# j-moralejo-pinas/dist_classicrl

Hardware: AMD Instinct MI355X
Metric: env-steps/sec at 128 agents, 1e6x16 Q-table; 1/2/4/8 GPU + HBM GB/s %peak (higher is better)
Workload: dtype f32

## Files before the change

### dist_classicrl_amd/csrc/qe_inst_lane.hip

```cpp
#include "qe_host.h"
#include "qe_rollout_df.h"

#if !defined(QE_INST_T) || !defined(QE_INST_ENV)
#error "compile with -DQE_INST_T=<float|double> -DQE_INST_ENV=<HashEnv|GridEnv|BanditEnv|TttEnv|TableEnv>"
#endif

template <int NV, int CAP, bool MK, int LEAN, bool HELP, bool FULL, bool SEQ>
constexpr int64_t lane_variant() {
    return QE_VARIANT_PERSISTENT | ((int64_t)LEAN << 4) | ((int64_t)HELP << 6) | ((int64_t)FULL << 7) | ((int64_t)SEQ << 8) |
           ((int64_t)(CAP == LANE_MAX_AGENTS) << 9) | ((int64_t)NV << 12) | ((int64_t)MK << 20);
}

template <typename T, class Env>
int launch_persistent(qe_engine* e, qe_env* env, RolloutSlot& sl, const Ctx<T>& c, const EnvCtx& ev, int64_t steps, int mode,
                      int build) {
    const unsigned block = (unsigned)((env->N + 63) / 64 * 64);
    int flags = FLAG_ACCOUNT;
#ifdef QE_EXPERIMENT
    if (getenv("QE_DEBUG_FLAGS")) flags |= atoi(getenv("QE_DEBUG_FLAGS")) << 20;
#endif
    const bool lean = mode == QE_LEARN_ITER && !c.trace && !c.rp.s;
    auto go = [&](auto nv, auto masked) {
        constexpr int NV = decltype(nv)::value;
        constexpr bool MK = decltype(masked)::value;
        constexpr bool HAS_LEAN = std::is_same<T, float>::value &&
                                  ((std::is_same<Env, HashEnv>::value && !MK && (NV == 2 || NV == 4)) ||
                                   std::is_same<Env, TttEnv>::value);
        const bool full = (int64_t)block == env->N;
        const bool light = build == 1, sparse = build == 3;
        auto launch = [&](auto cap, auto lean_c, auto help, auto full_c, auto seq, unsigned threads) {
            constexpr int CAP = decltype(cap)::value, LEAN = decltype(lean_c)::value;
            constexpr bool HELP = decltype(help)::value, FULL = decltype(full_c)::value, SEQ = decltype(seq)::value;
            hipLaunchKernelGGL((k_rollout_lane<T, Env, NV, CAP, MK, LEAN, HELP, FULL, SEQ>), dim3(1), dim3(threads), 0, e->stream,
                               sl.sched, c, ev, (long long)steps, flags);
            sl.variant = lane_variant<NV, CAP, MK, LEAN, HELP, FULL, SEQ>();
        };
        auto launch_df = [&](auto lean_c, auto full_c) {
            constexpr int LEAN = decltype(lean_c)::value;
            constexpr bool FULL = decltype(full_c)::value;
            if constexpr (LEAN != 0) {
                hipLaunchKernelGGL((k_rollout_df<T, Env, NV, MK, LEAN, FULL>), dim3(1), dim3(2 * block), 0, e->stream,
                                   sl.sched, c, ev, (long long)steps, flags);
                sl.variant = lane_variant<NV, 128, MK, LEAN, true, FULL, true>() | QE_VARIANT_DATAFLOW;
            }
        };
        using I128 = std::integral_constant<int, 128>;
        using I512 = std::integral_constant<int, LANE_MAX_AGENTS>;
        using L0 = std::integral_constant<int, 0>;
        using L1 = std::integral_constant<int, HAS_LEAN ? 1 : 0>;
        using L2 = std::integral_constant<int, HAS_LEAN ? 2 : 0>;
        using Y = std::integral_constant<bool, HAS_LEAN>;
        using N = std::false_type;
        auto by_lean = [&](auto f) { if (c.dlog) f(L2{}); else f(L1{}); };
        if (HAS_LEAN && lean && block <= 128) {
            if (full && sparse) by_lean([&](auto l) { launch(I128{}, l, Y{}, Y{}, Y{}, 2 * block); });
            else if (full && light) by_lean([&](auto l) { launch_df(l, Y{}); });
            else if (light) by_lean([&](auto l) { launch_df(l, N{}); });
            else if (full) by_lean([&](auto l) { launch(I128{}, l, Y{}, Y{}, N{}, std::max(512u, 2 * block)); });
            else by_lean([&](auto l) { launch(I128{}, l, Y{}, N{}, N{}, std::max(512u, 2 * block)); });
        } else {
            launch(I512{}, L0{}, N{}, N{}, N{}, block);
        }
    };
    using Yes = std::true_type;
    using No = std::false_type;
    if constexpr (std::is_same<Env, HashEnv>::value || std::is_same<Env, TableEnv>::value) {
        auto by_mask = [&](auto nv) { if (env->p.masked) go(nv, Yes{}); else go(nv, No{}); };
        switch (e->ld) {
            case 4: by_mask(std::integral_constant<int, 1>{}); break;
            case 8: by_mask(std::integral_constant<int, 2>{}); break;
            case 16: by_mask(std::integral_constant<int, 4>{}); break;
            case 32: by_mask(std::integral_constant<int, 8>{}); break;
            default: by_mask(std::integral_constant<int, 16>{}); break;
        }
    } else if constexpr (std::is_same<Env, TttEnv>::value) {
        go(std::integral_constant<int, 4>{}, Yes{});
    } else {
        go(std::integral_constant<int, 1>{}, No{});
    }
    ++sl.launches;
    return QE_OK;
}

template int launch_persistent<QE_INST_T, QE_INST_ENV>(qe_engine*, qe_env*, RolloutSlot&, const Ctx<QE_INST_T>&, const EnvCtx&, int64_t, int,
                                                       int);
```

### dist_classicrl_amd/csrc/qe_rollout_lane.h

```cpp
#pragma once
#include "qe_kernels.h"

namespace qe {

constexpr int LANE_MAX_AGENTS = 512;

template <typename T, int NV>
struct RowV {
    T v[4 * NV];
};

template <int NV>
struct LaneMask {
    using type = uint32_t;
};
template <>
struct LaneMask<16> {
    using type = uint64_t;
};

__device__ __forceinline__ int popc_mask(uint32_t x) { return __popc(x); }
__device__ __forceinline__ int popc_mask(uint64_t x) { return __popcll(x); }

template <int NV>
__device__ __forceinline__ void load_row_lane(RowV<float, NV>& r, const float* q, int64_t row) {
    const float4* p = reinterpret_cast<const float4*>(q + row * (4 * NV));
#pragma unroll
    for (int k = 0; k < NV; ++k) {
        const float4 f = p[k];
        r.v[4 * k] = f.x; r.v[4 * k + 1] = f.y; r.v[4 * k + 2] = f.z; r.v[4 * k + 3] = f.w;
    }
}
template <int NV>
__device__ __forceinline__ void load_row_lane(RowV<double, NV>& r, const double* q, int64_t row) {
    const double2* p = reinterpret_cast<const double2*>(q + row * (4 * NV));
#pragma unroll
    for (int k = 0; k < NV; ++k) {
        const double2 a = p[2 * k], b = p[2 * k + 1];
        r.v[4 * k] = a.x; r.v[4 * k + 1] = a.y; r.v[4 * k + 2] = b.x; r.v[4 * k + 3] = b.y;
    }
}

__device__ __forceinline__ float lane_fmax(float a, float b) { return __builtin_fmaxf(a, b); }
__device__ __forceinline__ double lane_fmax(double a, double b) { return __builtin_fmax(a, b); }

template <bool MASKED, typename T, int NV, typename M>
__device__ __forceinline__ RowV<T, NV> masked_row(const RowV<T, NV>& row, M valid) {
    if constexpr (!MASKED) {
        return row;
    } else {
        RowV<T, NV> r;
#pragma unroll
        for (int j = 0; j < 4 * NV; ++j) r.v[j] = ((valid >> j) & 1) ? row.v[j] : neg_inf<T>();
        return r;
    }
}

template <typename T, int NV>
__device__ __forceinline__ T row_max_lane(const RowV<T, NV>& rowm) {
    T m = neg_inf<T>();
#pragma unroll
    for (int j = 0; j < 4 * NV; ++j) m = lane_fmax(m, rowm.v[j]);
    return m;
}

template <int NV>
__device__ __forceinline__ bool row_nan_lane(const RowV<float, NV>& rowm) {
    typedef float f2 __attribute__((ext_vector_type(2)));
    f2 acc0 = {0.0f, 0.0f}, acc1 = {0.0f, 0.0f};
#pragma unroll
    for (int j = 0; j < 4 * NV; j += 4) {
        const f2 x = {rowm.v[j], rowm.v[j + 1]}, y = {rowm.v[j + 2], rowm.v[j + 3]};
        acc0 = __builtin_elementwise_fma(x, x, acc0);
        acc1 = __builtin_elementwise_fma(y, y, acc1);
    }
    const f2 acc = acc0 + acc1;
    const float s = acc.x + acc.y;
    return s != s;
}
template <int NV>
__device__ __forceinline__ bool row_nan_lane(const RowV<double, NV>& rowm) {
    double acc = 0.0;
#pragma unroll
    for (int j = 0; j < 4 * NV; ++j) acc += rowm.v[j] * rowm.v[j];
    return acc != acc;
}
template <typename T, int NV>
__device__ __forceinline__ T row_max_np_lane(const RowV<T, NV>& rowm) {
    const T m = row_max_lane(rowm);
    return row_nan_lane<NV>(rowm) ? quiet_nan<T>() : m;
}

template <typename T, int NV, int LO, int CNT>
__device__ __forceinline__ T row_pick_tree(const RowV<T, NV>& row, int idx) {
    constexpr int W = 4 * NV;
    if constexpr (CNT == 1) {
        T x = row.v[LO < W ? LO : W - 1];
        asm volatile("" : "+v"(x));
        return x;
    } else {
        const T lo = row_pick_tree<T, NV, LO, CNT / 2>(row, idx);
        const T hi = row_pick_tree<T, NV, LO + CNT / 2, CNT / 2>(row, idx);
        T r = (idx & (CNT / 2)) ? hi : lo;
        asm volatile("" : "+v"(r));
        return r;
    }
}
template <typename T, int NV>
__device__ __forceinline__ T row_pick_lane(const RowV<T, NV>& row, int idx) {
    constexpr int W = 4 * NV;
    constexpr int P = W <= 4 ? 4 : (W <= 8 ? 8 : (W <= 16 ? 16 : (W <= 32 ? 32 : 64)));
    return row_pick_tree<T, NV, 0, P>(row, idx);
}

template <int NV, typename M>
__device__ __forceinline__ int kth_set_bit(M f, int k) {
    constexpr int W = 4 * NV;
    constexpr int P = W <= 4 ? 4 : (W <= 8 ? 8 : (W <= 16 ? 16 : (W <= 32 ? 32 : 64)));
    constexpr int LOG = P == 4 ? 2 : (P == 8 ? 3 : (P == 16 ? 4 : (P == 32 ? 5 : 6)));
    int pos = 0;
#pragma unroll
    for (int lv = 0; lv < LOG; ++lv) {
        const int width = P >> (lv + 1);
        const M low = f & (((M)1 << width) - 1);
        const int c = popc_mask(low);
        const bool hi = k >= c;
        k -= hi ? c : 0;
        f = hi ? (f >> width) : low;
        pos += hi ? width : 0;
    }
    return pos;
}

template <typename T, int NV, typename M>
__device__ __forceinline__ int select_lane(const RowV<T, NV>& rowm, M valid, bool explore, uint32_t x1,
                                           uint32_t x2, T* picked, bool nan_max) {
    T m = row_max_lane(rowm);
    if (nan_max) m = quiet_nan<T>();
    M ties = 0;
#pragma unroll
    for (int j = 0; j < 4 * NV; ++j) ties |= (M)(rowm.v[j] == m ? 1u : 0u) << j;
    const M f = explore ? valid : (ties & valid);
    const int total = popc_mask(f);
    int act = -1;
    if (total > 0) act = kth_set_bit<NV>(f, (int)mulhi32(explore ? x1 : x2, (uint32_t)total));
    *picked = row_pick_lane(rowm, act < 0 ? 0 : act);
    return act;
}

template <class Env, int NV, bool MASKED>
__device__ __forceinline__ typename LaneMask<NV>::type valid_mask_lane(const EnvCtx& ev, int64_t i, int32_t obs) {
    using M = typename LaneMask<NV>::type;
    if constexpr (!MASKED) {
        return ev.A >= 8 * (int)sizeof(M) ? ~(M)0 : (((M)1 << ev.A) - 1);
    } else {
        M m = 0;
#pragma unroll
        for (int sub = 0; sub < NV; ++sub) m |= (M)Env::valid4(ev, i, obs, sub) << (4 * sub);
        return m;
    }
}

template <int CAP>
struct LaneCfg {
    static constexpr int WT = CAP <= 128 ? 4096 : 2048;
    static constexpr int BT = 2048;
};

template <int CAP, bool HELP>
struct LaneLds {
    SlowLdsT<CAP, PERSIST_CACHE_BYTES> slow;
    int wt[4][LaneCfg<CAP>::WT + 1];
    int bt_key[LaneCfg<CAP>::BT];
    unsigned bt_cnt[LaneCfg<CAP>::BT];
    int bt_min[LaneCfg<CAP>::BT];
    uint32_t draws[2][3][HELP ? CAP : 1];
    unsigned long long ep_key[EP_STAGE];
    float ep_ret[EP_STAGE];
    unsigned char pending[CAP];
    alignas(16) unsigned char cold[448];
    unsigned def_bits[CAP / 32];
    unsigned busy[5];
    unsigned ep_n;
    unsigned n_def;
    unsigned complex_;
    int seq_min[2];
};

#ifdef QE_EXPERIMENT
#define QX(bit) ((flags >> (20 + (bit))) & 1)
#else
#define QX(bit) 0
#endif
#ifdef QE_STAMPS
#define QL_STAMP(k) do { const long long _n = wall_clock64(); stamp_sum[k] += _n - stamp_last; stamp_last = _n; } while (0)
#else
#define QL_STAMP(k) do { } while (0)
#endif

template <int PENDING_LOADS>
__device__ __forceinline__ void step_barrier() {
    if constexpr (PENDING_LOADS == 0) asm volatile("s_waitcnt vmcnt(0) lgkmcnt(0)\n\ts_barrier" ::: "memory");
    else asm volatile("s_waitcnt vmcnt(%0) lgkmcnt(0)\n\ts_barrier" ::"n"(PENDING_LOADS) : "memory");
}

template <typename T, class Env, int NV, int CAP, bool MASKED, int LEAN = 0, bool HELP = false, bool FULL = false,
          bool SEQ = false>
__global__ __launch_bounds__(HELP ? 4 * CAP : CAP) void k_rollout_lane(InlineSched ,
                                                                       Ctx<T> c, EnvCtx ev, long long steps, int flags) {
    using M = typename LaneMask<NV>::type;
    constexpr int NLOAD = NV * (int)(sizeof(T) / 4);
    constexpr int WT = LaneCfg<CAP>::WT, BT = LaneCfg<CAP>::BT;
    __shared__ LaneLds<CAP, HELP> lds;
    const unsigned long long clk0 = wall_clock64();
    const unsigned long long cyc0 = __builtin_amdgcn_s_memtime();
    if (c.thr == nullptr) {
        const QE_AS4 unsigned char* ka = (const QE_AS4 unsigned char*)__builtin_amdgcn_kernarg_segment_ptr();
        c.thr = (const QE_AS4 unsigned long long*)ka;
        c.lr = (const QE_AS4 double*)(ka + sizeof(unsigned long long) * INLINE_SCHED_STEPS);
    }
    if constexpr (LEAN != 0) { c.mode = 0; c.trace = nullptr; c.rp.s = nullptr; }
    if constexpr (LEAN == 1) c.dlog = nullptr;
#ifdef QE_STAMPS
    long long stamp_sum[8] = {0, 0, 0, 0, 0, 0, 0, 0};
    long long stamp_last = wall_clock64();
    if (threadIdx.x == 0) for (int k = 8; k < 24; ++k) c.vinc[k] = 0.0;
#endif
    const int tid = threadIdx.x;
    const int n_main = HELP ? (int)((c.N + 63) & ~63ll) : (int)blockDim.x;
    const int wave_tid = __builtin_amdgcn_readfirstlane(tid);
    const bool helper = HELP && wave_tid >= n_main && wave_tid < 2 * n_main;
    const bool worker = HELP && wave_tid >= 2 * n_main;
    const int i = helper ? tid - n_main : (worker ? 0 : tid);
    const bool active = FULL ? !(helper || worker) : (!(helper || worker) && i < c.N);
    const int ii = i < c.N ? i : 0;
    Pending<T> p;
    p.n = c.n[ii];
    p.aux = c.aux[ii];
    p.s = 0; p.a = 0; p.pred = 0; p.r = 0.0f; p.term = false;
    float acc = c.acc[ii];
    unsigned long long deferred_total = 0, ep_base = 0;
    unsigned complex_steps = 0;
    int w_next = WT, w_cur = WT, w_prev = WT;
    const int flush_every = 32;
    int flush_in = flush_every;
    for (int k = tid; k < 4 * (WT + 1); k += (int)blockDim.x) (&lds.wt[0][0])[k] = -1;
    for (int k = tid; k < BT; k += (int)blockDim.x) { lds.bt_key[k] = -1; lds.bt_cnt[k] = 0u; lds.bt_min[k] = 0x7FFFFFFF; }
    for (int k = tid; k < CAP; k += (int)blockDim.x) lds.pending[k] = 0;
    if (tid < CAP / 32) lds.def_bits[tid] = 0u;
    static_assert(sizeof(Ctx<T>) <= sizeof(lds.cold), "context stash too small");
    if (tid == 0) {
        *reinterpret_cast<Ctx<T>*>(lds.cold) = c;
        lds.ep_n = 0u; lds.n_def = 0u; lds.complex_ = 0u;
        lds.seq_min[0] = 0x7FFFFFFF; lds.seq_min[1] = 0x7FFFFFFF;
        for (int k = 0; k < 5; ++k) lds.busy[k] = 0u;
        c.ctrl->error = 0u;
        c.ctrl->inv_count = 0u;
    }
    __syncthreads();
    if ((QX(6) && worker) || (QX(7) && helper)) return;

    const bool nan_sel = c.nan_select != 0;
    auto advance = [&](const RowV<T, NV>& row, M valid, long long t1, const U4& x, unsigned long long thr_t1, bool row_nan) {
        const bool explore = (unsigned long long)x.x < thr_t1;
        T picked;
        int act = select_lane<T, NV, M>(masked_row<MASKED>(row, valid), valid, explore, x.y, x.z, &picked, nan_sel && row_nan);
        if (act < 0) {
            c.ctrl->error = ERR_EMPTY_CHOICE;
            act = 0;
        }
        const int32_t n = p.n;
        const Transition tr = Env::step(ev, i, n, p.aux, act, c.step0 + (unsigned long long)t1);
        if (c.trace) c.trace[t1 * c.N + i] = act;
        replay_put(c, t1, i, n, act, tr.reward, tr.next_obs, tr.terminated);
        p.s = n; p.a = act; p.pred = picked; p.r = tr.reward; p.term = tr.terminated; p.n = tr.next_obs;
    };
    auto philox_of = [&](long long t1) {
        const unsigned long long step1 = c.step0 + (unsigned long long)t1;
        return philox4x32_10(c.agent_offset + (uint32_t)ii, (uint32_t)step1, (uint32_t)(step1 >> 32), STREAM_POLICY,
                             c.seed_lo, c.seed_hi);
    };
    auto draws = [&](long long t1) {
        if constexpr (HELP) {
            const int slot = (int)(t1 & 1);
            return U4{lds.draws[slot][0][ii], lds.draws[slot][1][ii], lds.draws[slot][2][ii], 0u};
        } else {
            return philox_of(t1);
        }
    };
    auto produce = [&](long long t1) {
        const U4 x = philox_of(t1);
        const int slot = (int)(t1 & 1);
        lds.draws[slot][0][ii] = x.x; lds.draws[slot][1][ii] = x.y; lds.draws[slot][2][ii] = x.z;
    };
    auto bookkeeping = [&](long long k, bool check_stale) {
        int* const tab_w = lds.wt[(k + 1) & 3];
        const int* const tab_r = lds.wt[k & 3];
        const int* const tab_st = lds.wt[(k + 3) & 3];
        const int32_t rowid = p.n;
        const int h = (int)(mix32((uint32_t)rowid) & (WT - 1));
        const bool need_r = rowid != p.s;
        int o_w = atomicCAS(&tab_w[h], -1, rowid);
        int k_r = need_r ? tab_r[h] : -1;
        int k_st = check_stale ? tab_st[h] : -1;
        int h_w = h, h_r = h, h_st = h;
        bool odd_w = o_w != -1 && o_w != rowid, odd_r = k_r != -1 && k_r != rowid, odd_st = k_st != -1 && k_st != rowid;
        while (__any(odd_w || odd_r || odd_st)) {
            h_w = odd_w ? (h_w + 1) & (WT - 1) : h_w;
            h_r = (h_r + 1) & (WT - 1);
            h_st = (h_st + 1) & (WT - 1);
            const int o2 = atomicCAS(&tab_w[odd_w ? h_w : WT], odd_w ? -1 : -2, rowid);
            const int r2 = tab_r[odd_r ? h_r : WT];
            const int s2 = tab_st[odd_st ? h_st : WT];
            o_w = odd_w ? o2 : o_w; k_r = odd_r ? r2 : k_r; k_st = odd_st ? s2 : k_st;
            odd_w = o_w != -1 && o_w != rowid; odd_r = k_r != -1 && k_r != rowid; odd_st = k_st != -1 && k_st != rowid;
        }
        lds.busy[o_w == rowid ? (int)((k + 1) & 3) : 4] = 1u;
        lds.busy[k_r == rowid ? (int)(k & 3) : 4] = 1u;
        w_prev = w_cur; w_cur = w_next; w_next = h_w;
        return k_st == rowid;
    };

    RowV<T, NV> row;
    bool stale = false;
    {
        load_row_lane<NV>(row, c.q, p.n);
        if (active) {
            const M valid0 = valid_mask_lane<Env, NV, MASKED>(ev, i, p.n);
            advance(row, valid0, 0, philox_of(0), c.thr[0], row_nan_lane<NV>(masked_row<MASKED>(row, valid0)));
            int h = (int)(mix32((uint32_t)p.s) & (WT - 1));
            int old = atomicCAS(&lds.wt[0][h], -1, p.s);
            while (old != -1 && old != p.s) {
                h = (h + 1) & (WT - 1);
                old = atomicCAS(&lds.wt[0][h], -1, p.s);
            }
            if (old == p.s) lds.busy[0] = 1u;
            w_next = h;
        }
        if (helper) produce(1);
        __syncthreads();
        if (active) (void)bookkeeping(0, false);
        load_row_lane<NV>(row, c.q, p.n);
    }
    __syncthreads();
    DeltaEntry* dl = c.dlog ? c.dlog + c.dlog_base + ii : nullptr;
    const long long dl_steps = c.dlog ? (c.dlog_cap - c.dlog_base) / c.N : 0;
    int vzero;
    asm volatile("v_mov_b32 %0, 0" : "=v"(vzero));
    double lr_pend = ((const double*)(uintptr_t)c.lr)[vzero];
    unsigned long long thr_pend = ((const unsigned long long*)(uintptr_t)c.thr)[(steps > 1 ? 1 : 0) + vzero];
    for (long long t = 0; t < steps; ++t) {
        const bool last = t + 1 == steps;
        const bool dl_ok = t < dl_steps;
        QL_STAMP(7);
        const bool busy = lds.busy[t & 3] != 0u;
        const U4 x = draws(t + 1);
        if (helper && !last && !QX(5)) produce(t + 2);
        if (stale && !QX(8)) load_row_lane<NV>(row, c.q, p.n);
        const M valid = valid_mask_lane<Env, NV, MASKED>(ev, ii, p.n);
        QL_STAMP(0);
        int cls = 3;
        int pred_s = -1, pred_n = -1;
        int b_s = -1, b_n = -1;
        if (busy) {
            if (active) {
                auto bt_insert = [&](int32_t rowid) {
                    int h = (int)(mix32((uint32_t)rowid) & (BT - 1));
                    for (;;) {
                        const int old = atomicCAS(&lds.bt_key[h], -1, rowid);
                        if (old == -1 || old == rowid) return h;
                        h = (h + 1) & (BT - 1);
                    }
                };
                b_s = bt_insert(p.s);
                atomicAdd(&lds.bt_cnt[b_s], 1u << 16);
                atomicMin(&lds.bt_min[b_s], i);
                if (p.n != p.s) {
                    b_n = bt_insert(p.n);
                    atomicAdd(&lds.bt_cnt[b_n], 1u);
                    atomicMin(&lds.bt_min[b_n], i);
                }
            }
            barrier_lds();
            if (active) {
                const unsigned cs = lds.bt_cnt[b_s];
                const int ms = lds.bt_min[b_s];
                unsigned cn = 0u;
                int mn = 0x7FFFFFFF;
                const bool has_n = b_n >= 0;
                if (has_n) { cn = lds.bt_cnt[b_n]; mn = lds.bt_min[b_n]; }
                const unsigned w_s = cs >> 16, tot_s = w_s + (cs & 0xFFFFu);
                const unsigned w_n = cn >> 16, tot_n = w_n + (cn & 0xFFFFu);
                bool now = true, sel = true, cx = false;
                if (c.mode == 1) {
                    const bool shared = w_s >= 2u || (w_s == 1u && tot_s >= 2u) || (has_n && w_n >= 1u && tot_n >= 2u);
                    if (shared) { now = false; cx = true; }
                    sel = !(has_n ? w_n > 0u : w_s > 1u);
                } else {
                    if (tot_s > 1u && ms < i) { now = false; pred_s = ms; cx |= tot_s > 2u; }
                    if (has_n) {
                        if (w_n > 0u) {
                            sel = false;
                            if (!p.term && mn < i) { now = false; pred_n = mn; cx |= tot_n > 2u; }
                        }
                    } else if (w_s > 1u) {
                        sel = false;
                    }
                }
                cls = (now ? 1 : 0) | (sel ? 2 : 0);
                if (!now) {
                    lds.pending[i] = 1;
                    atomicAdd(&lds.n_def, 1u);
                    if (cx) lds.complex_ = 1u;
                }
            }
        }
        QL_STAMP(2);
        __builtin_amdgcn_s_waitcnt(0x0F70);
        double lr_t;
        unsigned long long thr_t1;
        asm volatile("v_mov_b64 %0, %1" : "=v"(lr_t) : "v"(lr_pend));
        asm volatile("v_mov_b64 %0, %1" : "=v"(thr_t1) : "v"(thr_pend));
        lr_pend = ((const double*)(uintptr_t)c.lr)[(last ? t : t + 1) + vzero];
        thr_pend = ((const unsigned long long*)(uintptr_t)c.thr)[(t + 2 < steps ? t + 2 : steps - 1) + vzero];
        const float r_t = p.r;
        const bool term_t = p.term;
        bool row_nan = row_nan_lane<NV>(masked_row<MASKED>(row, valid));
        if (active && (cls & 1)) {
            T m = row_max_lane(masked_row<MASKED>(row, valid));
            if (row_nan) m = quiet_nan<T>();
            const int64_t cell = (int64_t)p.s * (4 * NV) + p.a;
            T u;
            const T q1 = Td<T>::apply(p.pred, p.r, m, p.term, make_hyper(c, lr_t), c.mode, &u);
            if (p.n == p.s) row_nan |= q1 != q1;
            if (!QX(1)) c.q[cell] = q1;
            if (dl_ok) *dl = DeltaEntry{(uint32_t)cell, (float)u};
            if (p.n == p.s) {
#pragma unroll
                for (int j = 0; j < 4 * NV; ++j) row.v[j] = j == p.a ? q1 : row.v[j];
            }
        }
        unsigned ep_raw = 0;
        unsigned long long enders = 0;
        float ep_value = 0.0f;
        if (active) {
            acc += r_t;
            enders = __ballot(term_t && (flags & FLAG_ACCOUNT));
            const unsigned rank = __builtin_amdgcn_mbcnt_hi((unsigned)(enders >> 32), __builtin_amdgcn_mbcnt_lo((unsigned)enders, 0u));
            if (term_t) {
                if (rank == 0) ep_raw = atomicAdd(&lds.ep_n, (unsigned)__popcll(enders));
                ep_value = acc;
                acc = 0.0f;
            }
        }
        QL_STAMP(4);
        if (active && !busy && !last) advance(row, valid, t + 1, x, thr_t1, row_nan);
        QL_STAMP(5);

        if (busy) {
#ifdef QE_STAMPS
            const long long ext_t0 = wall_clock64();
#endif
            __syncthreads();
            const int n_def = (int)lds.n_def;
            if (active) {
                lds.bt_key[b_s] = -1; lds.bt_cnt[b_s] = 0u; lds.bt_min[b_s] = 0x7FFFFFFF;
                if (b_n >= 0) { lds.bt_key[b_n] = -1; lds.bt_cnt[b_n] = 0u; lds.bt_min[b_n] = 0x7FFFFFFF; }
            }
#ifdef QE_STAMPS
            if (tid == 0) { c.vinc[16] += 1.0; if (n_def > 0) c.vinc[17] += 1.0; }
#endif
            if (n_def > 0) {
                deferred_total += (unsigned long long)n_def;
                if (lds.complex_) ++complex_steps;
                if constexpr (SEQ) if (lds.complex_) {
                    bool mine = active && !(cls & 1);
                    for (int round = 0; round <= n_def; ++round) {
                        if (mine) atomicMin(&lds.seq_min[round & 1], i);
                        barrier_lds();
                        const int turn = lds.seq_min[round & 1];
                        if (tid == 0) lds.seq_min[(round + 1) & 1] = 0x7FFFFFFF;
                        if (turn == 0x7FFFFFFF) break;
                        if (mine && i == turn) {
                            T m = 0;
                            if (!p.term) {
                                RowV<T, NV> fresh;
                                load_row_lane<NV>(fresh, c.q, p.n);
                                m = row_max_np_lane<T, NV>(masked_row<MASKED>(fresh, valid));
                            }
                            const int64_t cell = (int64_t)p.s * (4 * NV) + p.a;
                            const T q0 = c.q[cell];
                            T u;
                            c.q[cell] = Td<T>::apply(q0, p.r, m, p.term, make_hyper(c, lr_t), 0, &u);
                            log_delta(c, t, i, cell, u);
                            lds.pending[i] = 0;
                            mine = false;
                        }
                        __syncthreads();
                    }
                    if (tid == 0) { lds.seq_min[0] = 0x7FFFFFFF; lds.seq_min[1] = 0x7FFFFFFF; }
                }
                if (!SEQ && lds.complex_) {
                    const Ctx<T>& cold = *reinterpret_cast<const Ctx<T>*>(lds.cold);
                    Ctx<T> cc = c;
                    cc.s = cold.s; cc.a = cold.a; cc.n = cold.n; cc.r = cold.r; cc.term = cold.term;
                    cc.pred = cold.pred; cc.aux = cold.aux; cc.acc = cold.acc;
                    cc.inv_bitmap = cold.inv_bitmap; cc.inv_list = cold.inv_list; cc.vinc = cold.vinc;
                    cc.ctrl = cold.ctrl; cc.ep_key = cold.ep_key; cc.ep_ret = cold.ep_ret; cc.ep_cap = cold.ep_cap;
                    cc.stamps = nullptr; cc.tok = nullptr; cc.adv_bitmap = nullptr; cc.pend_list = nullptr;
                    const bool mine_def = active && !(cls & 1);
                    if (c.mode == 0) {
                        if (mine_def) atomicOr(&lds.def_bits[i >> 5], 1u << (i & 31));
                        barrier_lds();
                        if (mine_def) {
                            int pos = __popc(lds.def_bits[i >> 5] & ((1u << (i & 31)) - 1u));
                            for (int w = 0; w < (i >> 5); ++w) pos += __popc(lds.def_bits[w]);
                            lds.slow.a_agent[pos] = i; lds.slow.a_s[pos] = p.s; lds.slow.a_a[pos] = p.a;
                            lds.slow.a_n[pos] = p.n; lds.slow.a_r[pos] = p.r; lds.slow.a_term[pos] = p.term ? 1 : 0;
                            lds.pending[i] = 0;
                        }
                        barrier_lds();
                        if (tid < CAP / 32) lds.def_bits[tid] = 0u;
                        slow_body<T, Env, CAP, PERSIST_CACHE_BYTES, NV>(
                            cc, ev, FLAG_NO_STAMPS | FLAG_LEARN | FLAG_PRESTAGED, t, n_def, lds.slow);
                    } else {
                        if (mine_def) {
                            cc.s[i] = p.s; cc.a[i] = p.a; cc.pred[i] = p.pred; cc.r[i] = p.r;
                            cc.term[i] = p.term ? 1 : 0; cc.n[i] = p.n; cc.aux[i] = p.aux;
                            atomicOr(&cc.inv_bitmap[i >> 5], 1u << (i & 31));
                            lds.pending[i] = 0;
                        }
                        __syncthreads();
                        (void)build_involved_list(cc, lds.slow.scan);
                        slow_body<T, Env, CAP, PERSIST_CACHE_BYTES, NV>(cc, ev, FLAG_NO_STAMPS | FLAG_LEARN, t, n_def, lds.slow);
                    }
                    __syncthreads();
                } else if (!lds.complex_) {
                    bool mine = active && !(cls & 1);
                    int rounds = 0;
                    while (lds.n_def > 0u && rounds++ <= n_def) {
#ifdef QE_STAMPS
                        if (tid == 0) c.vinc[18] += 1.0;
#endif
                        const bool go = mine && (pred_s < 0 || lds.pending[pred_s] == 0) &&
                                        (pred_n < 0 || lds.pending[pred_n] == 0);
                        barrier_lds();
                        if (go) {
                            T m = 0;
                            if (!p.term) {
                                RowV<T, NV> fresh;
                                load_row_lane<NV>(fresh, c.q, p.n);
                                m = row_max_np_lane<T, NV>(masked_row<MASKED>(fresh, valid));
                            }
                            const int64_t cell = (int64_t)p.s * (4 * NV) + p.a;
                            const T q0 = c.q[cell];
                            T u;
                            c.q[cell] = Td<T>::apply(q0, p.r, m, p.term, make_hyper(c, lr_t), 0, &u);
                            log_delta(c, t, i, cell, u);
                            lds.pending[i] = 0;
                            atomicSub(&lds.n_def, 1u);
                            mine = false;
                        }
                        __syncthreads();
                    }
                    if (tid == 0 && lds.n_def > 0u) reinterpret_cast<const Ctx<T>*>(lds.cold)->ctrl->error = 2u;
                }
            }
            if (active && !last) {
                if (cls != 3 && !((cls & 2) && p.n != p.s)) load_row_lane<NV>(row, c.q, p.n);
                advance(row, valid, t + 1, x, thr_t1, row_nan_lane<NV>(masked_row<MASKED>(row, valid)));
            }
            if (tid == 0) { lds.n_def = 0u; lds.complex_ = 0u; }
            __builtin_amdgcn_s_waitcnt(0x0F70);
#ifdef QE_STAMPS
            if (tid == 0) c.vinc[19] += (double)(wall_clock64() - ext_t0);
#endif
        }
        if (enders) {
            const unsigned base = __builtin_amdgcn_readlane(ep_raw, __ffsll((long long)enders) - 1);
            if ((enders >> (threadIdx.x & 63)) & 1) {
                const unsigned ep_slot = base + __builtin_amdgcn_mbcnt_hi((unsigned)(enders >> 32),
                                                                          __builtin_amdgcn_mbcnt_lo((unsigned)enders, 0u));
                const unsigned long long key = ((unsigned long long)t << 32) | (unsigned long long)i;
                if (ep_slot < (unsigned)EP_STAGE) {
                    lds.ep_key[ep_slot] = key;
                    lds.ep_ret[ep_slot] = ep_value;
                } else {
                    asm volatile("" ::: "memory");
                    const Ctx<T>& cc = *reinterpret_cast<const Ctx<T>*>(lds.cold);
                    if ((long long)(ep_base + ep_slot) < cc.ep_cap) {
                        cc.ep_key[ep_base + ep_slot] = key;
                        cc.ep_ret[ep_base + ep_slot] = ep_value;
                    }
                }
            }
        }
        if (--flush_in == 0 || last) {
            flush_in = flush_every;
            __syncthreads();
            const unsigned staged = lds.ep_n;
            const Ctx<T>& cc = *reinterpret_cast<const Ctx<T>*>(lds.cold);
            unsigned long long* const out_key = cc.ep_key;
            float* const out_ret = cc.ep_ret;
            const long long out_cap = cc.ep_cap;
            for (unsigned k = tid; k < min(staged, (unsigned)EP_STAGE); k += blockDim.x) {
                const unsigned long long pos = ep_base + k;
                if ((long long)pos < out_cap) { out_key[pos] = lds.ep_key[k]; out_ret[pos] = lds.ep_ret[k]; }
            }
            ep_base += staged;
            __syncthreads();
            if (tid == 0) lds.ep_n = 0u;
        }
        QL_STAMP(6);
        if (last) break;
        lds.wt[(t + 3) & 3][w_prev] = -1;
        if (tid == 0) lds.busy[(t + 3) & 3] = 0u;
        asm volatile("" ::: "memory");
        if (!helper && !worker && !QX(0)) load_row_lane<NV>(row, c.q, p.n);
        asm volatile("" ::: "memory");
        if (active && !QX(2)) stale = bookkeeping(t + 1, true);
        QL_STAMP(1);
        if (!QX(4)) step_barrier<NLOAD>();
        if (c.dlog) dl += c.N;
    }
#ifdef QE_STAMPS
    if (tid == 0 && c.vinc) for (int k = 0; k < 8; ++k) c.vinc[k] = (double)stamp_sum[k];
#endif
    const Ctx<T>& cc = *reinterpret_cast<const Ctx<T>*>(lds.cold);
    if (active) {
        cc.n[i] = p.n; cc.aux[i] = p.aux; cc.acc[i] = acc;
        if (cc.hb) { cc.hb_obs[i] = p.n; cc.hb_aux[i] = p.aux; cc.hb_acc[i] = acc; }
    }
    if (tid == 0) {
        cc.ctrl->involved_total = deferred_total;
        cc.ctrl->pending_total = complex_steps;
        cc.ctrl->ep_count = ep_base;
        cc.ctrl->t_local = steps;
    }
    if (cc.hb) {
        asm volatile("s_waitcnt vmcnt(0)" ::: "memory");
        __syncthreads();
        if (tid == 0) {
            HostBlock* hb = cc.hb;
            hb->ep_count = ep_base;
            hb->involved_total = deferred_total;
            hb->error = cc.ctrl->error;
            hb->complex_steps = complex_steps;
            hb->clk0 = clk0;
            hb->clk1 = wall_clock64();
            hb->cyc0 = cyc0;
            hb->cyc1 = __builtin_amdgcn_s_memtime();
            __threadfence_system();
            asm volatile("s_waitcnt vmcnt(0)" ::: "memory");
            __hip_atomic_store(&hb->seq, cc.hb_seq, __ATOMIC_RELEASE, __HIP_MEMORY_SCOPE_SYSTEM);
        }
    }
}

}
```

Before: 29.42 million.

## Restructure lane rollout step: hoist row max/NaN, asm tie mask, prefetch picked Q value

Reorders the per-step loop of the persistent lane kernel. The row max and NaN sum are computed once early, and episode accounting and the LDS atomic are moved before the TD update so their latency overlaps other work. Tie detection uses inline-asm compare and carry chains, and the picked Q value is loaded from global memory with the next row instead of being extracted from registers. LDS draws are packed as vectors, and the step counter is narrowed to int with a new guard on step count. The cost is added inline-asm fragility, an extra outstanding load in the barrier count, and hand-written waitcnt ordering.

After: 28.77 million. 2.2% lower.

```diff
diff --git a/dist_classicrl_amd/csrc/qe_inst_lane.hip b/dist_classicrl_amd/csrc/qe_inst_lane.hip
--- a/dist_classicrl_amd/csrc/qe_inst_lane.hip
+++ b/dist_classicrl_amd/csrc/qe_inst_lane.hip
@@ -14,6 +14,7 @@
 template <typename T, class Env>
 int launch_persistent(qe_engine* e, qe_env* env, RolloutSlot& sl, const Ctx<T>& c, const EnvCtx& ev, int64_t steps, int mode,
                       int build) {
+    if (steps > 0x7FFFFFFFll - 2) return QE_ERR_INVALID;
     const unsigned block = (unsigned)((env->N + 63) / 64 * 64);
     int flags = FLAG_ACCOUNT;
 #ifdef QE_EXPERIMENT
diff --git a/dist_classicrl_amd/csrc/qe_rollout_lane.h b/dist_classicrl_amd/csrc/qe_rollout_lane.h
--- a/dist_classicrl_amd/csrc/qe_rollout_lane.h
+++ b/dist_classicrl_amd/csrc/qe_rollout_lane.h
@@ -65,7 +65,7 @@
 }
 
 template <int NV>
-__device__ __forceinline__ bool row_nan_lane(const RowV<float, NV>& rowm) {
+__device__ __forceinline__ float row_nan_sum_lane(const RowV<float, NV>& rowm) {
     typedef float f2 __attribute__((ext_vector_type(2)));
     f2 acc0 = {0.0f, 0.0f}, acc1 = {0.0f, 0.0f};
 #pragma unroll
@@ -75,15 +75,19 @@
         acc1 = __builtin_elementwise_fma(y, y, acc1);
     }
     const f2 acc = acc0 + acc1;
-    const float s = acc.x + acc.y;
+    return acc.x + acc.y;
+}
+template <int NV>
+__device__ __forceinline__ double row_nan_sum_lane(const RowV<double, NV>& rowm) {
+    double acc = 0.0;
+#pragma unroll
+    for (int j = 0; j < 4 * NV; ++j) acc += rowm.v[j] * rowm.v[j];
+    return acc;
+}
+template <int NV, typename T>
+__device__ __forceinline__ bool row_nan_lane(const RowV<T, NV>& rowm) {
+    const T s = row_nan_sum_lane<NV>(rowm);
     return s != s;
-}
-template <int NV>
-__device__ __forceinline__ bool row_nan_lane(const RowV<double, NV>& rowm) {
-    double acc = 0.0;
-#pragma unroll
-    for (int j = 0; j < 4 * NV; ++j) acc += rowm.v[j] * rowm.v[j];
-    return acc != acc;
 }
 template <typename T, int NV>
 __device__ __forceinline__ T row_max_np_lane(const RowV<T, NV>& rowm) {
@@ -132,20 +136,50 @@
     return pos;
 }
 
+#define QE_TIE4_ASM(CMP)                                                                                                   \
+    asm(CMP "_e64 %3, %7, %8\n\t" CMP "_e64 %2, %6, %8\n\t" CMP "_e64 %1, %5, %8\n\t" CMP "_e32 vcc, %4, %8\n\t"           \
+        "v_addc_co_u32_e64 %0, %3, %0, %0, %3\n\tv_addc_co_u32_e64 %0, %2, %0, %0, %2\n\t"                                 \
+        "v_addc_co_u32_e64 %0, %1, %0, %0, %1\n\tv_addc_co_u32_e32 %0, vcc, %0, %0, vcc"                                   \
+        : "+v"(acc), "=&s"(c1), "=&s"(c2), "=&s"(c3)                                                                       \
+        : "v"(v0), "v"(v1), "v"(v2), "v"(v3), "v"(m)                                                                       \
+        : "vcc")
+__device__ __forceinline__ uint32_t tie4_lane(uint32_t acc, float v0, float v1, float v2, float v3, float m) {
+    unsigned long long c1, c2, c3;
+    QE_TIE4_ASM("v_cmp_eq_f32");
+    return acc;
+}
+__device__ __forceinline__ uint32_t tie4_lane(uint32_t acc, double v0, double v1, double v2, double v3, double m) {
+    unsigned long long c1, c2, c3;
+    QE_TIE4_ASM("v_cmp_eq_f64");
+    return acc;
+}
+#undef QE_TIE4_ASM
+template <typename T, int NV, typename M>
+__device__ __forceinline__ M tie_mask_lane(const RowV<T, NV>& r, T m) {
+    uint32_t acc[NV > 8 ? 2 : 1] = {};
+#pragma unroll
+    for (int k = NV - 1; k >= 0; --k)
+        acc[k / 8] = tie4_lane(acc[k / 8], r.v[4 * k], r.v[4 * k + 1], r.v[4 * k + 2], r.v[4 * k + 3], m);
+    if constexpr (NV > 8) return (M)acc[0] | ((M)acc[1] << 32);
+    else return (M)acc[0];
+}
+
 template <typename T, int NV, typename M>
 __device__ __forceinline__ int select_lane(const RowV<T, NV>& rowm, M valid, bool explore, uint32_t x1,
-                                           uint32_t x2, T* picked, bool nan_max) {
-    T m = row_max_lane(rowm);
+                                           uint32_t x2, T* picked, bool nan_max, T m) {
     if (nan_max) m = quiet_nan<T>();
-    M ties = 0;
-#pragma unroll
-    for (int j = 0; j < 4 * NV; ++j) ties |= (M)(rowm.v[j] == m ? 1u : 0u) << j;
+    const M ties = tie_mask_lane<T, NV, M>(rowm, m);
     const M f = explore ? valid : (ties & valid);
     const int total = popc_mask(f);
     int act = -1;
     if (total > 0) act = kth_set_bit<NV>(f, (int)mulhi32(explore ? x1 : x2, (uint32_t)total));
-    *picked = row_pick_lane(rowm, act < 0 ? 0 : act);
+    if (picked) *picked = row_pick_lane(rowm, act < 0 ? 0 : act);
     return act;
+}
+template <typename T, int NV, typename M>
+__device__ __forceinline__ int select_lane(const RowV<T, NV>& rowm, M valid, bool explore, uint32_t x1,
+                                           uint32_t x2, T* picked, bool nan_max) {
+    return select_lane<T, NV, M>(rowm, valid, explore, x1, x2, picked, nan_max, row_max_lane(rowm));
 }
 
 template <class Env, int NV, bool MASKED>
@@ -174,7 +208,7 @@
     int bt_key[LaneCfg<CAP>::BT];
     unsigned bt_cnt[LaneCfg<CAP>::BT];
     int bt_min[LaneCfg<CAP>::BT];
-    uint32_t draws[2][3][HELP ? CAP : 1];
+    alignas(16) uint32_t draws[2][HELP ? CAP : 1][4];
     unsigned long long ep_key[EP_STAGE];
     float ep_ret[EP_STAGE];
     unsigned char pending[CAP];
@@ -260,11 +294,17 @@
     __syncthreads();
     if ((QX(6) && worker) || (QX(7) && helper)) return;
 
+    constexpr bool CARRY_LOAD = LEAN != 0 && !MASKED;
+    auto load_pred = [&]() {
+        if constexpr (CARRY_LOAD) p.pred = c.q[(int64_t)p.s * (4 * NV) + p.a];
+    };
     const bool nan_sel = c.nan_select != 0;
-    auto advance = [&](const RowV<T, NV>& row, M valid, long long t1, const U4& x, unsigned long long thr_t1, bool row_nan) {
+    auto advance = [&](const RowV<T, NV>& row, M valid, long long t1, const U4& x, unsigned long long thr_t1, bool row_nan,
+                       T row_max) {
         const bool explore = (unsigned long long)x.x < thr_t1;
-        T picked;
-        int act = select_lane<T, NV, M>(masked_row<MASKED>(row, valid), valid, explore, x.y, x.z, &picked, nan_sel && row_nan);
+        T picked = p.pred;
+        int act = select_lane<T, NV, M>(masked_row<MASKED>(row, valid), valid, explore, x.y, x.z, CARRY_LOAD ? nullptr : &picked,
+                                        nan_sel && row_nan, row_max);
         if (act < 0) {
             c.ctrl->error = ERR_EMPTY_CHOICE;
             act = 0;
@@ -280,10 +320,12 @@
         return philox4x32_10(c.agent_offset + (uint32_t)ii, (uint32_t)step1, (uint32_t)(step1 >> 32), STREAM_POLICY,
                              c.seed_lo, c.seed_hi);
     };
+    typedef uint32_t DrawV __attribute__((ext_vector_type(3)));
     auto draws = [&](long long t1) {
         if constexpr (HELP) {
             const int slot = (int)(t1 & 1);
-            return U4{lds.draws[slot][0][ii], lds.draws[slot][1][ii], lds.draws[slot][2][ii], 0u};
+            const DrawV d = *reinterpret_cast<const DrawV*>(lds.draws[slot][ii]);
+            return U4{d.x, d.y, d.z, 0u};
         } else {
             return philox_of(t1);
         }
@@ -291,7 +333,7 @@
     auto produce = [&](long long t1) {
         const U4 x = philox_of(t1);
         const int slot = (int)(t1 & 1);
-        lds.draws[slot][0][ii] = x.x; lds.draws[slot][1][ii] = x.y; lds.draws[slot][2][ii] = x.z;
+        *reinterpret_cast<DrawV*>(lds.draws[slot][ii]) = DrawV{x.x, x.y, x.z};
     };
     auto bookkeeping = [&](long long k, bool check_stale) {
         int* const tab_w = lds.wt[(k + 1) & 3];
@@ -327,7 +369,8 @@
         load_row_lane<NV>(row, c.q, p.n);
         if (active) {
             const M valid0 = valid_mask_lane<Env, NV, MASKED>(ev, i, p.n);
-            advance(row, valid0, 0, philox_of(0), c.thr[0], row_nan_lane<NV>(masked_row<MASKED>(row, valid0)));
+            advance(row, valid0, 0, philox_of(0), c.thr[0], row_nan_lane<NV>(masked_row<MASKED>(row, valid0)),
+                    row_max_lane(masked_row<MASKED>(row, valid0)));
             int h = (int)(mix32((uint32_t)p.s) & (WT - 1));
             int old = atomicCAS(&lds.wt[0][h], -1, p.s);
             while (old != -1 && old != p.s) {
@@ -341,24 +384,58 @@
         __syncthreads();
         if (active) (void)bookkeeping(0, false);
         load_row_lane<NV>(row, c.q, p.n);
+        load_pred();
     }
     __syncthreads();
     DeltaEntry* dl = c.dlog ? c.dlog + c.dlog_base + ii : nullptr;
-    const long long dl_steps = c.dlog ? (c.dlog_cap - c.dlog_base) / c.N : 0;
+    const int nsteps = (int)steps;
+    const long long dl_fit = c.dlog ? (c.dlog_cap - c.dlog_base) / c.N : 0;
+    const int dl_steps = dl_fit < (long long)nsteps ? (int)dl_fit : nsteps;
+    typedef __attribute__((address_space(3))) unsigned LdsWord;
+    LdsWord* ep_n_ptr = (LdsWord*)&lds.ep_n;
+    asm volatile("" : "+v"(ep_n_ptr));
     int vzero;
     asm volatile("v_mov_b32 %0, 0" : "=v"(vzero));
     double lr_pend = ((const double*)(uintptr_t)c.lr)[vzero];
-    unsigned long long thr_pend = ((const unsigned long long*)(uintptr_t)c.thr)[(steps > 1 ? 1 : 0) + vzero];
-    for (long long t = 0; t < steps; ++t) {
-        const bool last = t + 1 == steps;
+    unsigned long long thr_pend = ((const unsigned long long*)(uintptr_t)c.thr)[(nsteps > 1 ? 1 : 0) + vzero];
+    for (int t = 0; t < nsteps; ++t) {
+        const bool last = t + 1 == nsteps;
         const bool dl_ok = t < dl_steps;
         QL_STAMP(7);
-        const bool busy = lds.busy[t & 3] != 0u;
+        unsigned busy_word = lds.busy[t & 3];
         const U4 x = draws(t + 1);
         if (helper && !last && !QX(5)) produce(t + 2);
         if (stale && !QX(8)) load_row_lane<NV>(row, c.q, p.n);
         const M valid = valid_mask_lane<Env, NV, MASKED>(ev, ii, p.n);
         QL_STAMP(0);
+        __builtin_amdgcn_s_waitcnt(0x0F70);
+        double lr_t;
+        unsigned long long thr_t1;
+        asm volatile("v_mov_b64 %0, %1" : "=v"(lr_t) : "v"(lr_pend));
+        asm volatile("v_mov_b64 %0, %1" : "=v"(thr_t1) : "v"(thr_pend));
+        lr_pend = ((const double*)(uintptr_t)c.lr)[(last ? t : t + 1) + vzero];
+        thr_pend = ((const unsigned long long*)(uintptr_t)c.thr)[(t + 2 < nsteps ? t + 2 : nsteps - 1) + vzero];
+        const T nan_sum = row_nan_sum_lane<NV>(masked_row<MASKED>(row, valid));
+        T row_max = row_max_lane(masked_row<MASKED>(row, valid));
+        asm volatile("" : "+v"(busy_word) : "v"(nan_sum), "v"(row_max));
+        const bool busy = __builtin_amdgcn_readfirstlane(busy_word) != 0u;
+        bool row_nan = nan_sum != nan_sum;
+        const float r_t = p.r;
+        const bool term_t = p.term;
+        unsigned ep_raw = 0;
+        unsigned long long enders = 0;
+        float ep_value = 0.0f;
+        if (active) {
+            acc += r_t;
+            enders = __ballot(term_t && (flags & FLAG_ACCOUNT));
+            const unsigned rank = __builtin_amdgcn_mbcnt_hi((unsigned)(enders >> 32), __builtin_amdgcn_mbcnt_lo((unsigned)enders, 0u));
+            if (term_t) {
+                if (rank == 0)
+                    ep_raw = __hip_atomic_fetch_add(ep_n_ptr, (unsigned)__popcll(enders), __ATOMIC_RELAXED, __HIP_MEMORY_SCOPE_WORKGROUP);
+                ep_value = acc;
+                acc = 0.0f;
+            }
+        }
         int cls = 3;
         int pred_s = -1, pred_n = -1;
         int b_s = -1, b_n = -1;
@@ -416,19 +493,8 @@
             }
         }
         QL_STAMP(2);
-        __builtin_amdgcn_s_waitcnt(0x0F70);
-        double lr_t;
-        unsigned long long thr_t1;
-        asm volatile("v_mov_b64 %0, %1" : "=v"(lr_t) : "v"(lr_pend));
-        asm volatile("v_mov_b64 %0, %1" : "=v"(thr_t1) : "v"(thr_pend));
-        lr_pend = ((const double*)(uintptr_t)c.lr)[(last ? t : t + 1) + vzero];
-        thr_pend = ((const unsigned long long*)(uintptr_t)c.thr)[(t + 2 < steps ? t + 2 : steps - 1) + vzero];
-        const float r_t = p.r;
-        const bool term_t = p.term;
-        bool row_nan = row_nan_lane<NV>(masked_row<MASKED>(row, valid));
         if (active && (cls & 1)) {
-            T m = row_max_lane(masked_row<MASKED>(row, valid));
-            if (row_nan) m = quiet_nan<T>();
+            const T m = row_nan ? quiet_nan<T>() : row_max;
             const int64_t cell = (int64_t)p.s * (4 * NV) + p.a;
             T u;
             const T q1 = Td<T>::apply(p.pred, p.r, m, p.term, make_hyper(c, lr_t), c.mode, &u);
@@ -438,23 +504,11 @@
             if (p.n == p.s) {
 #pragma unroll
                 for (int j = 0; j < 4 * NV; ++j) row.v[j] = j == p.a ? q1 : row.v[j];
-            }
-        }
-        unsigned ep_raw = 0;
-        unsigned long long enders = 0;
-        float ep_value = 0.0f;
-        if (active) {
-            acc += r_t;
-            enders = __ballot(term_t && (flags & FLAG_ACCOUNT));
-            const unsigned rank = __builtin_amdgcn_mbcnt_hi((unsigned)(enders >> 32), __builtin_amdgcn_mbcnt_lo((unsigned)enders, 0u));
-            if (term_t) {
-                if (rank == 0) ep_raw = atomicAdd(&lds.ep_n, (unsigned)__popcll(enders));
-                ep_value = acc;
-                acc = 0.0f;
+                row_max = row_max_lane(masked_row<MASKED>(row, valid));
             }
         }
         QL_STAMP(4);
-        if (active && !busy && !last) advance(row, valid, t + 1, x, thr_t1, row_nan);
+        if (active && !busy && !last) advance(row, valid, t + 1, x, thr_t1, row_nan, row_max);
         QL_STAMP(5);
 
         if (busy) {
@@ -568,7 +622,8 @@
             }
             if (active && !last) {
                 if (cls != 3 && !((cls & 2) && p.n != p.s)) load_row_lane<NV>(row, c.q, p.n);
-                advance(row, valid, t + 1, x, thr_t1, row_nan_lane<NV>(masked_row<MASKED>(row, valid)));
+                advance(row, valid, t + 1, x, thr_t1, row_nan_lane<NV>(masked_row<MASKED>(row, valid)),
+                        row_max_lane(masked_row<MASKED>(row, valid)));
             }
             if (tid == 0) { lds.n_def = 0u; lds.complex_ = 0u; }
             __builtin_amdgcn_s_waitcnt(0x0F70);
@@ -577,6 +632,7 @@
 #endif
         }
         if (enders) {
+            __builtin_amdgcn_s_waitcnt(0xC07F);
             const unsigned base = __builtin_amdgcn_readlane(ep_raw, __ffsll((long long)enders) - 1);
             if ((enders >> (threadIdx.x & 63)) & 1) {
                 const unsigned ep_slot = base + __builtin_amdgcn_mbcnt_hi((unsigned)(enders >> 32),
@@ -616,11 +672,15 @@
         lds.wt[(t + 3) & 3][w_prev] = -1;
         if (tid == 0) lds.busy[(t + 3) & 3] = 0u;
         asm volatile("" ::: "memory");
-        if (!helper && !worker && !QX(0)) load_row_lane<NV>(row, c.q, p.n);
+        if (!helper && !worker && !QX(0)) {
+            load_row_lane<NV>(row, c.q, p.n);
+            load_pred();
+        }
         asm volatile("" ::: "memory");
         if (active && !QX(2)) stale = bookkeeping(t + 1, true);
         QL_STAMP(1);
-        if (!QX(4)) step_barrier<NLOAD>();
+        asm volatile("" ::"v"(ep_raw), "v"(x.x), "v"(x.y), "v"(x.z));
+        if (!QX(4)) step_barrier<NLOAD + (CARRY_LOAD ? 1 : 0)>();
         if (c.dlog) dl += c.N;
     }
 #ifdef QE_STAMPS
```

## Offload schedule loads, episode accounting and pred reload to helper waves

Applied to the files above, without the earlier changes.

In the slim variant (helper waves, sequential, full, lean), helper waves now stage the per-step learning rate and epsilon threshold into an LDS ring and take over episode-return accounting from reward/terminal pairs the main lanes write to LDS. Main lanes drop their per-step global loads of lr/thr and the ballot/atomic accounting. They also re-read the predicted Q value from memory one step ahead instead of extracting it from the row, and the barrier allows one extra outstanding load. The aim is a shorter critical path per step on the main waves, at the cost of more LDS traffic and more complex coupling between helper and main waves.

Measured after the change: 27.75 million before, 30.27 million after (median of 6 runs). 1.09x the previous value.

```diff
diff --git a/dist_classicrl_amd/csrc/qe_rollout_lane.h b/dist_classicrl_amd/csrc/qe_rollout_lane.h
--- a/dist_classicrl_amd/csrc/qe_rollout_lane.h
+++ b/dist_classicrl_amd/csrc/qe_rollout_lane.h
@@ -132,7 +132,7 @@
     return pos;
 }
 
-template <typename T, int NV, typename M>
+template <typename T, int NV, typename M, bool PICK = true>
 __device__ __forceinline__ int select_lane(const RowV<T, NV>& rowm, M valid, bool explore, uint32_t x1,
                                            uint32_t x2, T* picked, bool nan_max) {
     T m = row_max_lane(rowm);
@@ -144,7 +144,7 @@
     const int total = popc_mask(f);
     int act = -1;
     if (total > 0) act = kth_set_bit<NV>(f, (int)mulhi32(explore ? x1 : x2, (uint32_t)total));
-    *picked = row_pick_lane(rowm, act < 0 ? 0 : act);
+    if constexpr (PICK) *picked = row_pick_lane(rowm, act < 0 ? 0 : act);
     return act;
 }
 
@@ -187,6 +187,27 @@
     int seq_min[2];
 };
 
+struct alignas(16) SchedSlot {
+    double lr;
+    unsigned long long thr;
+};
+template <int CAP>
+struct LaneLdsSlim : LaneLds<CAP, true> {
+    SchedSlot sched[2];
+    uint2 acct[2][CAP];
+};
+
+__device__ __forceinline__ float opaque_copy(float v) {
+    float r;
+    asm volatile("v_mov_b32 %0, %1" : "=v"(r) : "v"(v));
+    return r;
+}
+__device__ __forceinline__ double opaque_copy(double v) {
+    double r;
+    asm volatile("v_mov_b64 %0, %1" : "=v"(r) : "v"(v));
+    return r;
+}
+
 #ifdef QE_EXPERIMENT
 #define QX(bit) ((flags >> (20 + (bit))) & 1)
 #else
@@ -211,7 +232,8 @@
     using M = typename LaneMask<NV>::type;
     constexpr int NLOAD = NV * (int)(sizeof(T) / 4);
     constexpr int WT = LaneCfg<CAP>::WT, BT = LaneCfg<CAP>::BT;
-    __shared__ LaneLds<CAP, HELP> lds;
+    constexpr bool SLIM = HELP && SEQ && FULL && LEAN != 0;
+    __shared__ std::conditional_t<SLIM, LaneLdsSlim<CAP>, LaneLds<CAP, HELP>> lds;
     const unsigned long long clk0 = wall_clock64();
     const unsigned long long cyc0 = __builtin_amdgcn_s_memtime();
     if (c.thr == nullptr) {
@@ -263,8 +285,8 @@
     const bool nan_sel = c.nan_select != 0;
     auto advance = [&](const RowV<T, NV>& row, M valid, long long t1, const U4& x, unsigned long long thr_t1, bool row_nan) {
         const bool explore = (unsigned long long)x.x < thr_t1;
-        T picked;
-        int act = select_lane<T, NV, M>(masked_row<MASKED>(row, valid), valid, explore, x.y, x.z, &picked, nan_sel && row_nan);
+        T picked = p.pred;
+        int act = select_lane<T, NV, M, !SLIM>(masked_row<MASKED>(row, valid), valid, explore, x.y, x.z, &picked, nan_sel && row_nan);
         if (act < 0) {
             c.ctrl->error = ERR_EMPTY_CHOICE;
             act = 0;
@@ -292,6 +314,43 @@
         const U4 x = philox_of(t1);
         const int slot = (int)(t1 & 1);
         lds.draws[slot][0][ii] = x.x; lds.draws[slot][1][ii] = x.y; lds.draws[slot][2][ii] = x.z;
+        if constexpr (SLIM) {
+            if (tid == n_main) {
+                lds.sched[slot].lr = c.lr[t1 - 1];
+                lds.sched[slot].thr = c.thr[t1 < steps ? t1 : (steps > 0 ? steps - 1 : 0)];
+            }
+        }
+    };
+    auto helper_account = [&](long long tk) {
+        if constexpr (SLIM) {
+            const uint2 rt = lds.acct[tk & 1][ii];
+            const bool term = rt.y != 0u;
+            acc += __uint_as_float(rt.x);
+            const bool ends = term && (flags & FLAG_ACCOUNT);
+            const unsigned long long enders = __ballot(ends);
+            const float ep_value = acc;
+            if (term) acc = 0.0f;
+            if (enders) {
+                const unsigned rank = __builtin_amdgcn_mbcnt_hi((unsigned)(enders >> 32), __builtin_amdgcn_mbcnt_lo((unsigned)enders, 0u));
+                unsigned ep_raw = 0;
+                if (ends && rank == 0) ep_raw = atomicAdd(&lds.ep_n, (unsigned)__popcll(enders));
+                const unsigned base = __builtin_amdgcn_readlane(ep_raw, __ffsll((long long)enders) - 1);
+                if (ends) {
+                    const unsigned ep_slot = base + rank;
+                    const unsigned long long key = ((unsigned long long)tk << 32) | (unsigned long long)ii;
+                    if (ep_slot < (unsigned)EP_STAGE) {
+                        lds.ep_key[ep_slot] = key;
+                        lds.ep_ret[ep_slot] = ep_value;
+                    } else {
+                        const Ctx<T>& cc = *reinterpret_cast<const Ctx<T>*>(lds.cold);
+                        if ((long long)(ep_base + ep_slot) < cc.ep_cap) {
+                            cc.ep_key[ep_base + ep_slot] = key;
+                            cc.ep_ret[ep_base + ep_slot] = ep_value;
+                        }
+                    }
+                }
+            }
+        }
     };
     auto bookkeeping = [&](long long k, bool check_stale) {
         int* const tab_w = lds.wt[(k + 1) & 3];
@@ -323,6 +382,8 @@
 
     RowV<T, NV> row;
     bool stale = false;
+    T* pred_cell = c.q;
+    T pred_pend = 0;
     {
         load_row_lane<NV>(row, c.q, p.n);
         if (active) {
@@ -341,21 +402,34 @@
         __syncthreads();
         if (active) (void)bookkeeping(0, false);
         load_row_lane<NV>(row, c.q, p.n);
+        if constexpr (SLIM) {
+            pred_cell = c.q + ((int64_t)p.s * (4 * NV) + p.a);
+            pred_pend = *pred_cell;
+        }
+        if constexpr (SLIM) if (active) lds.acct[0][i] = make_uint2(__float_as_uint(p.r), p.term ? 1u : 0u);
     }
     __syncthreads();
     DeltaEntry* dl = c.dlog ? c.dlog + c.dlog_base + ii : nullptr;
     const long long dl_steps = c.dlog ? (c.dlog_cap - c.dlog_base) / c.N : 0;
-    int vzero;
-    asm volatile("v_mov_b32 %0, 0" : "=v"(vzero));
-    double lr_pend = ((const double*)(uintptr_t)c.lr)[vzero];
-    unsigned long long thr_pend = ((const unsigned long long*)(uintptr_t)c.thr)[(steps > 1 ? 1 : 0) + vzero];
+    int vzero = 0;
+    if constexpr (!SLIM) asm volatile("v_mov_b32 %0, 0" : "=v"(vzero));
+    double lr_pend = 0.0;
+    unsigned long long thr_pend = 0;
+    if constexpr (!SLIM) {
+        lr_pend = ((const double*)(uintptr_t)c.lr)[vzero];
+        thr_pend = ((const unsigned long long*)(uintptr_t)c.thr)[(steps > 1 ? 1 : 0) + vzero];
+    }
     for (long long t = 0; t < steps; ++t) {
         const bool last = t + 1 == steps;
         const bool dl_ok = t < dl_steps;
         QL_STAMP(7);
         const bool busy = lds.busy[t & 3] != 0u;
         const U4 x = draws(t + 1);
+        double lr_ring = 0.0;
+        unsigned long long thr_ring = 0;
+        if constexpr (SLIM) { lr_ring = lds.sched[(t + 1) & 1].lr; thr_ring = lds.sched[(t + 1) & 1].thr; }
         if (helper && !last && !QX(5)) produce(t + 2);
+        if constexpr (SLIM) if (helper) helper_account(t);
         if (stale && !QX(8)) load_row_lane<NV>(row, c.q, p.n);
         const M valid = valid_mask_lane<Env, NV, MASKED>(ev, ii, p.n);
         QL_STAMP(0);
@@ -419,10 +493,16 @@
         __builtin_amdgcn_s_waitcnt(0x0F70);
         double lr_t;
         unsigned long long thr_t1;
-        asm volatile("v_mov_b64 %0, %1" : "=v"(lr_t) : "v"(lr_pend));
-        asm volatile("v_mov_b64 %0, %1" : "=v"(thr_t1) : "v"(thr_pend));
-        lr_pend = ((const double*)(uintptr_t)c.lr)[(last ? t : t + 1) + vzero];
-        thr_pend = ((const unsigned long long*)(uintptr_t)c.thr)[(t + 2 < steps ? t + 2 : steps - 1) + vzero];
+        if constexpr (SLIM) {
+            lr_t = lr_ring;
+            thr_t1 = thr_ring;
+        } else {
+            asm volatile("v_mov_b64 %0, %1" : "=v"(lr_t) : "v"(lr_pend));
+            asm volatile("v_mov_b64 %0, %1" : "=v"(thr_t1) : "v"(thr_pend));
+            lr_pend = ((const double*)(uintptr_t)c.lr)[(last ? t : t + 1) + vzero];
+            thr_pend = ((const unsigned long long*)(uintptr_t)c.thr)[(t + 2 < steps ? t + 2 : steps - 1) + vzero];
+        }
+        if constexpr (SLIM) p.pred = opaque_copy(pred_pend);
         const float r_t = p.r;
         const bool term_t = p.term;
         bool row_nan = row_nan_lane<NV>(masked_row<MASKED>(row, valid));
@@ -433,7 +513,8 @@
             T u;
             const T q1 = Td<T>::apply(p.pred, p.r, m, p.term, make_hyper(c, lr_t), c.mode, &u);
             if (p.n == p.s) row_nan |= q1 != q1;
-            if (!QX(1)) c.q[cell] = q1;
+            if constexpr (SLIM) *pred_cell = q1;
+            else if (!QX(1)) c.q[cell] = q1;
             if (dl_ok) *dl = DeltaEntry{(uint32_t)cell, (float)u};
             if (p.n == p.s) {
 #pragma unroll
@@ -443,7 +524,7 @@
         unsigned ep_raw = 0;
         unsigned long long enders = 0;
         float ep_value = 0.0f;
-        if (active) {
+        if (!SLIM && active) {
             acc += r_t;
             enders = __ballot(term_t && (flags & FLAG_ACCOUNT));
             const unsigned rank = __builtin_amdgcn_mbcnt_hi((unsigned)(enders >> 32), __builtin_amdgcn_mbcnt_lo((unsigned)enders, 0u));
@@ -617,10 +698,17 @@
         if (tid == 0) lds.busy[(t + 3) & 3] = 0u;
         asm volatile("" ::: "memory");
         if (!helper && !worker && !QX(0)) load_row_lane<NV>(row, c.q, p.n);
+        if constexpr (SLIM) {
+            if (!helper && !worker) {
+                pred_cell = c.q + ((int64_t)p.s * (4 * NV) + p.a);
+                pred_pend = *pred_cell;
+            }
+        }
+        if constexpr (SLIM) if (active) lds.acct[(t + 1) & 1][i] = make_uint2(__float_as_uint(p.r), p.term ? 1u : 0u);
         asm volatile("" ::: "memory");
         if (active && !QX(2)) stale = bookkeeping(t + 1, true);
         QL_STAMP(1);
-        if (!QX(4)) step_barrier<NLOAD>();
+        if (!QX(4)) step_barrier<NLOAD + (SLIM ? 1 : 0)>();
         if (c.dlog) dl += c.N;
     }
 #ifdef QE_STAMPS
@@ -628,8 +716,16 @@
 #endif
     const Ctx<T>& cc = *reinterpret_cast<const Ctx<T>*>(lds.cold);
     if (active) {
-        cc.n[i] = p.n; cc.aux[i] = p.aux; cc.acc[i] = acc;
-        if (cc.hb) { cc.hb_obs[i] = p.n; cc.hb_aux[i] = p.aux; cc.hb_acc[i] = acc; }
+        cc.n[i] = p.n; cc.aux[i] = p.aux;
+        if constexpr (!SLIM) cc.acc[i] = acc;
+        if (cc.hb) {
+            cc.hb_obs[i] = p.n; cc.hb_aux[i] = p.aux;
+            if constexpr (!SLIM) cc.hb_acc[i] = acc;
+        }
+    }
+    if constexpr (SLIM) if (helper) {
+        cc.acc[ii] = acc;
+        if (cc.hb) cc.hb_acc[ii] = acc;
     }
     if (tid == 0) {
         cc.ctrl->involved_total = deferred_total;
```
